# azrael417/mlperf-deepcam

Measured on AMD Instinct MI355X. Metric: samples/sec (768x1152x16) train step, higher is better.
Workload: dtype bf16; 1 GPU; DeepLabV3+/Xception train step (fwd + weighted CE + bwd + LAMB), 768x1152x16, local_batch=8, bf16 activations / fp32 master weights, random-init seed 333; local_batch=8, global_batch=8, parallelism=dp1, optimizer=LAMB, hip_graph=False, launch_list_replay=False

## Files before the change

mlperf-deepcam_amd/csrc/dwpipe.hip:

```cpp
#include "common.h"
#include "dwtile.h"
#include "dwtile_common.h"
#include "bn_fin.h"
#include "mfma_tile.h"

namespace dc {

namespace {

constexpr int P_TH = 8, P_TW = 8, P_CG = 16, P_THREADS = 512;
constexpr int P_ROWB = P_CG * 16;
constexpr int P_CH = P_CG * 8;

enum { PM_FLIP = 1, PM_STATS = 2, PM_WGRAD = 4, PM_ADD = 8, PM_XFORM = 16, PM_RES = 32, PM_MASK = 64 };

template <int DIL>
struct PCfg {
  static constexpr int HH = P_TH + 2 * DIL, HW = P_TW + 2 * DIL, HP = HH * HW;
  static constexpr int HIT = (HP * P_CG + P_THREADS - 1) / P_THREADS;
  static constexpr int HALO = HIT * P_THREADS * 16;
  static constexpr int LASTW = (HP * P_CG - (HIT - 1) * P_THREADS + 63) / 64;
  static constexpr int TILE = P_TH * P_TW * P_ROWB;
};

template <int DIL, int MODE>
struct PStage {
  static constexpr bool Y = (MODE & (PM_STATS | PM_WGRAD)) != 0, A = (MODE & PM_ADD) != 0, Y2 = (MODE & PM_RES) != 0;
  static constexpr int BYTES = PCfg<DIL>::HALO + ((Y ? 1 : 0) + (Y2 ? 1 : 0) + (A ? 1 : 0)) * PCfg<DIL>::TILE;
  static constexpr int DMAS = PCfg<DIL>::HIT + 2 * ((Y ? 1 : 0) + (Y2 ? 1 : 0) + (A ? 1 : 0));
  static constexpr int OFF_Y2 = PCfg<DIL>::HALO + (Y ? PCfg<DIL>::TILE : 0), OFF_A = OFF_Y2 + (Y2 ? PCfg<DIL>::TILE : 0);
  static constexpr int NS = (160 * 1024 / BYTES) > 4 ? 4 : (160 * 1024 / BYTES);
  static constexpr int STORES = DT_PX;
  static_assert(NS >= 2, "the ring needs two stages");
  static_assert((NS - 1) * STORES + (NS - 2) * DMAS < 64, "vmcnt immediate");
};

struct DwpArgs {
  const bf16* in;
  int ldin;
  const float* wp;
  const bf16* addend;
  int ldadd;
  bf16* out;
  int ldout;
  int H, W, C;
  int ncb, ntx, nty, ptiles;
  const float* pscale;
  const float* pshift;
  int prelu;
  DwBnStats st;
  const bf16* y2;
  int ldy2;
  const float* mean2;
  const float* invstd2;
  int relu2;
  float* slab2;
  int sum_row, sum_row2;
};

template <int N>
__device__ inline void wait_vm() {
  asm volatile("s_waitcnt vmcnt(%0)" ::"n"(N) : "memory");
}

template <int DIL, int MODE>
__global__ __launch_bounds__(P_THREADS) void dwp_kernel(const DwpArgs a) {
  typedef PCfg<DIL> K;
  typedef PStage<DIL, MODE> S;
  constexpr bool FLIP = (MODE & PM_FLIP) != 0, STATS = (MODE & PM_STATS) != 0, WGRAD = (MODE & PM_WGRAD) != 0, ADD = (MODE & PM_ADD) != 0,
                 XFORM = (MODE & PM_XFORM) != 0, RES = (MODE & PM_RES) != 0, MASK = (MODE & PM_MASK) != 0;
  static_assert(!RES || (WGRAD && !STATS), "PM_RES rides on the weight-gradient form");
  static_assert(!MASK || RES, "PM_MASK is a form of PM_RES");
  constexpr int WC = DT_PX + 2 * DIL, KH = 4, NS = S::NS;
  extern __shared__ __attribute__((aligned(16))) char smem[];
  const int tid = threadIdx.x;
  const int wv = __builtin_amdgcn_readfirstlane(tid >> 6);
  const int cb = blockIdx.x % a.ncb, wj = blockIdx.x / a.ncb, wc = gridDim.x / a.ncb;
  const int t0 = (int)((long)a.ptiles * wj / wc), t1 = (int)((long)a.ptiles * (wj + 1) / wc);
  const int nt = t1 - t0;
  const int ngroups = a.C >> 3, cg0 = cb * P_CG;
  const int H = a.H, W = a.W;
  const int h = tid & 31, sl = tid >> 5;
  const int row = sl >> 1, xs = (sl & 1) * DT_PX;
  const bool cok = cg0 + (h >> 1) < ngroups;
  const int ch0 = cok ? cg0 * 8 + h * KH : 0;
  const int g = tid & 15;
  const bool gok = cg0 + g < ngroups;
  constexpr unsigned OOB = 0x80000000u;
  unsigned hoff[K::HIT];
  unsigned hedge = 0;
#pragma unroll
  for (int it = 0; it < K::HIT; ++it) {
    const int hp = (it * P_THREADS + tid) >> 4;
    const int hy = hp / K::HW, hx = hp - hy * K::HW;
    hoff[it] = (gok && hp < K::HP) ? (unsigned)((((hy - DIL) * W + (hx - DIL)) * a.ldin + (cg0 + g) * 8) * 2) : OOB;
    hedge |= ((hx < DIL ? 1u : 0u) | (hx >= K::HW - DIL ? 2u : 0u)) << (2 * it);
  }
  unsigned yoff[2], aoff[2], y2off[2];
#pragma unroll
  for (int it = 0; it < 2; ++it) {
    const int pp = (it * P_THREADS + tid) >> 4;
    const int py = pp >> 3, px = pp & 7;
    yoff[it] = gok && S::Y ? (unsigned)(((py * W + px) * a.st.ldy + (cg0 + g) * 8) * 2) : OOB;
    aoff[it] = gok && S::A ? (unsigned)(((py * W + px) * a.ldadd + (cg0 + g) * 8) * 2) : OOB;
    y2off[it] = gok && S::Y2 ? (unsigned)(((py * W + px) * a.ldy2 + (cg0 + g) * 8) * 2) : OOB;
  }

  auto issue = [&](int t, int stage) {
#if defined(__HIP_DEVICE_COMPILE__)
    char* sb = smem + stage * S::BYTES;
    const bool live = t < t1;
    const int tt = live ? t : t0;
    const int tx = tt % a.ntx;
    const int r = tt / a.ntx;
    const int ty = r % a.nty, n = r / a.nty;
    const int y0 = ty * P_TH, x0 = tx * P_TW;
    const int live_mask = live ? -1 : 0;
    const unsigned emask = (x0 == 0 ? 0x55555555u : 0u) | (x0 + P_TW == W ? 0xAAAAAAAAu : 0u);
    {
      const __amdgpu_buffer_rsrc_t rs = __builtin_amdgcn_make_buffer_rsrc((void*)(a.in + (size_t)n * H * W * a.ldin), 0, (H * W * a.ldin * 2) & live_mask, 0x00020000);
      const unsigned torg = (unsigned)((y0 * W + x0) * a.ldin * 2);
#pragma unroll
      for (int it = 0; it < K::HIT; ++it) {
        if (it == K::HIT - 1 && wv >= K::LASTW) break;
        const unsigned vo = ((hedge & emask) >> (2 * it)) & 3u ? OOB : hoff[it] + torg;
        __builtin_amdgcn_raw_ptr_buffer_load_lds(rs, (lds_ptr)(sb + (it * P_THREADS + wv * 64) * 16), 16, vo, 0, 0, 0);
      }
    }
    if constexpr (S::Y) {
      const __amdgpu_buffer_rsrc_t rs = __builtin_amdgcn_make_buffer_rsrc((void*)(reinterpret_cast<const bf16*>(a.st.y) + (size_t)n * H * W * a.st.ldy), 0,
                                                                          (H * W * a.st.ldy * 2) & live_mask, 0x00020000);
      const unsigned torg = (unsigned)((y0 * W + x0) * a.st.ldy * 2);
#pragma unroll
      for (int it = 0; it < 2; ++it)
        __builtin_amdgcn_raw_ptr_buffer_load_lds(rs, (lds_ptr)(sb + K::HALO + (it * P_THREADS + wv * 64) * 16), 16, yoff[it] + torg, 0, 0, 0);
    }
    if constexpr (S::A) {
      const __amdgpu_buffer_rsrc_t rs = __builtin_amdgcn_make_buffer_rsrc((void*)(a.addend + (size_t)n * H * W * a.ldadd), 0, (H * W * a.ldadd * 2) & live_mask, 0x00020000);
      const unsigned torg = (unsigned)((y0 * W + x0) * a.ldadd * 2);
#pragma unroll
      for (int it = 0; it < 2; ++it)
        __builtin_amdgcn_raw_ptr_buffer_load_lds(rs, (lds_ptr)(sb + S::OFF_A + (it * P_THREADS + wv * 64) * 16), 16, aoff[it] + torg, 0, 0, 0);
    }
    if constexpr (S::Y2) {
      const __amdgpu_buffer_rsrc_t rs = __builtin_amdgcn_make_buffer_rsrc((void*)(a.y2 + (size_t)n * H * W * a.ldy2), 0, (H * W * a.ldy2 * 2) & live_mask, 0x00020000);
      const unsigned torg = (unsigned)((y0 * W + x0) * a.ldy2 * 2);
#pragma unroll
      for (int it = 0; it < 2; ++it)
        __builtin_amdgcn_raw_ptr_buffer_load_lds(rs, (lds_ptr)(sb + S::OFF_Y2 + (it * P_THREADS + wv * 64) * 16), 16, y2off[it] + torg, 0, 0, 0);
    }
#endif
  };

#pragma unroll
  for (int s = 0; s < NS - 1; ++s) issue(t0 + s, s);

  float wk[9][KH];
  load_taps<KH>(a.wp, ch0, a.C, FLIP, wk);
  BnAcc<KH> bn;
  if constexpr (STATS) bn.init(a.st, ch0);
  else if constexpr (WGRAD) bn.init_affine(a.st, ch0);
  float dwa[WGRAD ? 9 : 1][KH];
#pragma unroll
  for (int t9 = 0; t9 < (WGRAD ? 9 : 1); ++t9)
#pragma unroll
    for (int e = 0; e < KH; ++e) dwa[t9][e] = 0.f;
  float mu2[RES ? KH : 1], is2[RES ? KH : 1], ra[RES ? KH : 1], rb[RES ? KH : 1];
  if constexpr (RES) {
#pragma unroll
    for (int e = 0; e < KH; ++e) {
      mu2[e] = a.mean2[ch0 + e];
      is2[e] = a.invstd2[ch0 + e];
      ra[e] = rb[e] = 0.f;
      asm volatile("" : "+v"(mu2[e]), "+v"(is2[e]));
    }
  }
  float xsc[8], xsh[8];
  if constexpr (XFORM) {
#pragma unroll
    for (int e = 0; e < 8; ++e) {
      xsc[e] = gok ? a.pscale[(cg0 + g) * 8 + e] : 0.f;
      xsh[e] = gok ? a.pshift[(cg0 + g) * 8 + e] : 0.f;
    }
  }
#pragma unroll
  for (int t9 = 0; t9 < 9; ++t9)
#pragma unroll
    for (int e = 0; e < KH; ++e) asm volatile("" : "+v"(wk[t9][e]));
  if constexpr (STATS || WGRAD) {
#pragma unroll
    for (int e = 0; e < KH; ++e) asm volatile("" : "+v"(bn.mu[e]), "+v"(bn.is[e]), "+v"(bn.ms[e]), "+v"(bn.mh[e]));
  }
  if constexpr (XFORM) {
#pragma unroll
    for (int e = 0; e < 8; ++e) asm volatile("" : "+v"(xsc[e]), "+v"(xsh[e]));
  }
  auto decode = [&](int t, int& n, int& y0, int& x0) {
    const int tx = t % a.ntx;
    const int r = t / a.ntx;
    const int ty = r % a.nty;
    n = r / a.nty;
    y0 = ty * P_TH;
    x0 = tx * P_TW;
  };
  auto xform_tile = [&](int t, int stg) {
    char* sb = smem + stg * S::BYTES;
    int n, y0, x0;
    decode(t, n, y0, x0);
    (void)n;
#pragma unroll
      for (int it = 0; it < K::HIT; ++it) {
        if (it == K::HIT - 1 && wv >= K::LASTW) break;
        const int hp = (it * P_THREADS + tid) >> 4;
        const int hy = hp / K::HW, hx = hp - hy * K::HW;
        const int iy = y0 - DIL + hy, ix = x0 - DIL + hx;
        if (gok && hp < K::HP && (unsigned)iy < (unsigned)H && (unsigned)ix < (unsigned)W) {
          vec16* q = reinterpret_cast<vec16*>(sb) + it * P_THREADS + tid;
          float f[8];
          unpack(*q, f, bf16());
#pragma unroll
          for (int e = 0; e < 8; ++e) {
            const float v = fmaf(f[e], xsc[e], xsh[e]);
            f[e] = a.prelu ? fmaxf(v, 0.f) : v;
          }
          vec16 o;
          pack(o, f, bf16());
          typedef unsigned u32x4 __attribute__((ext_vector_type(4)));
          u32x4 ov;
          ov.x = o.w[0]; ov.y = o.w[1]; ov.z = o.w[2]; ov.w = o.w[3];
          const unsigned qa = (unsigned)(size_t)((__attribute__((address_space(3))) char*)reinterpret_cast<char*>(q));
          asm volatile("ds_write_b128 %0, %1" ::"v"(qa), "v"(ov) : "memory");
        }
      }
  };
  auto compute_tile = [&](int t, int stg) {
    char* sb = smem + stg * S::BYTES;
    int n, y0, x0;
    decode(t, n, y0, x0);
    const char* tile = sb + h * 8;
    const int oy = y0 + row;
    float yf[DT_PX][KH];
    if constexpr (S::Y) {
#pragma unroll
      for (int j = 0; j < DT_PX; ++j)
        unpack8(*reinterpret_cast<const vec8*>(sb + K::HALO + (row * P_TW + xs + j) * P_ROWB + h * 8), yf[j], bf16());
    }
    float xh[WGRAD ? DT_PX : 1][KH];
    if constexpr (WGRAD) {
#pragma unroll
      for (int j = 0; j < DT_PX; ++j) {
        float v[KH];
#pragma unroll
        for (int e = 0; e < KH; ++e) {
          const float u = fmaf(yf[j][e], bn.ms[e], bn.mh[e]);
          v[e] = a.st.relu ? fmaxf(u, 0.f) : u;
        }
        vec8 rr;
        pack8(rr, v, bf16());
        unpack8(rr, xh[j], bf16());
      }
    }
    float acc[DT_PX][KH];
#pragma unroll
    for (int j = 0; j < DT_PX; ++j)
#pragma unroll
      for (int e = 0; e < KH; ++e) acc[j][e] = 0.f;
#pragma unroll
    for (int ky = 0; ky < 3; ++ky) {
#pragma unroll
      for (int c = 0; c < WC; ++c) {
        float f[KH];
        unpack8(*reinterpret_cast<const vec8*>(tile + ((row + ky * DIL) * K::HW + xs + c) * P_ROWB), f, bf16());
#pragma unroll
        for (int kx = 0; kx < 3; ++kx) {
          const int j = c - kx * DIL;
          if (j >= 0 && j < DT_PX) {
#pragma unroll
            for (int e = 0; e < KH; ++e) acc[j][e] = fmaf(f[e], wk[ky * 3 + kx][e], acc[j][e]);
            if constexpr (WGRAD) {
#pragma unroll
              for (int e = 0; e < KH; ++e) dwa[8 - (ky * 3 + kx)][e] = fmaf(f[e], xh[j][e], dwa[8 - (ky * 3 + kx)][e]);
            }
          }
        }
      }
    }
#pragma unroll
    for (int j = 0; j < DT_PX; ++j) {
      if constexpr (ADD) {
        float av[KH];
        unpack8(*reinterpret_cast<const vec8*>(sb + S::OFF_A + (row * P_TW + xs + j) * P_ROWB + h * 8), av, bf16());
#pragma unroll
        for (int e = 0; e < KH; ++e) acc[j][e] += av[e];
      }
      if constexpr (MASK) {
#pragma unroll
        for (int e = 0; e < KH; ++e) acc[j][e] = yf[j][e] > 0.f ? acc[j][e] : 0.f;
      }
      vec8 v;
      pack8(v, acc[j], bf16());
      if (cok) *reinterpret_cast<vec8*>(a.out + (((size_t)n * H + oy) * W + x0 + xs + j) * a.ldout + ch0) = v;
      if constexpr (STATS) {
        float gs[KH];
        unpack8(v, gs, bf16());
        bn.add(gs, yf[j], a.st.relu);
      }
      if constexpr (RES) {
        float gs[KH], y2f[KH];
        unpack8(v, gs, bf16());
        unpack8(*reinterpret_cast<const vec8*>(sb + S::OFF_Y2 + (row * P_TW + xs + j) * P_ROWB + h * 8), y2f, bf16());
#pragma unroll
        for (int e = 0; e < KH; ++e) {
          const float gm = (MASK || !a.relu2 || yf[j][e] > 0.f) ? gs[e] : 0.f;
          ra[e] += gm;
          rb[e] = fmaf(gm, (y2f[e] - mu2[e]) * is2[e], rb[e]);
        }
      }
    }
  };
  int stage = 0;
  if constexpr (!XFORM) {
    for (int i = 0; i < nt; ++i) {
      if (wv < K::LASTW) {
        if (i >= NS - 1) wait_vm<(NS - 1) * S::STORES + (NS - 2) * S::DMAS>();
        else if (i == 0) wait_vm<(NS - 2) * S::DMAS>();
        else if (i == 1) wait_vm<S::STORES + (NS - 2) * S::DMAS>();
        else wait_vm<2 * S::STORES + (NS - 2) * S::DMAS>();
      } else {
        if (i >= NS - 1) wait_vm<(NS - 1) * S::STORES + (NS - 2) * (S::DMAS - 1)>();
        else if (i == 0) wait_vm<(NS - 2) * (S::DMAS - 1)>();
        else if (i == 1) wait_vm<S::STORES + (NS - 2) * (S::DMAS - 1)>();
        else wait_vm<2 * S::STORES + (NS - 2) * (S::DMAS - 1)>();
      }
      __builtin_amdgcn_s_barrier();
      {
        int ns = stage + NS - 1;
        if (ns >= NS) ns -= NS;
        issue(t0 + i + NS - 1, ns);
      }
      compute_tile(t0 + i, stage);
      if (++stage == NS) stage = 0;
    }
  } else {
    static_assert(!XFORM || NS >= 3, "the transform one tile ahead needs three stages");
    constexpr int D0 = S::DMAS, D1 = S::DMAS - 1;
    if (wv < K::LASTW) wait_vm<(NS - 2) * D0>(); else wait_vm<(NS - 2) * D1>();
    __builtin_amdgcn_s_barrier();
    xform_tile(t0, 0);
    for (int i = 0; i < nt; ++i) {
      if (wv < K::LASTW) {
        if (i >= NS - 2) wait_vm<(NS - 2) * S::STORES + (NS - 3) * D0>();
        else if (i == 0) wait_vm<(NS - 3) * D0>();
        else wait_vm<S::STORES + (NS - 3) * D0>();
      } else {
        if (i >= NS - 2) wait_vm<(NS - 2) * S::STORES + (NS - 3) * D1>();
        else if (i == 0) wait_vm<(NS - 3) * D1>();
        else wait_vm<S::STORES + (NS - 3) * D1>();
      }
      asm volatile("s_waitcnt lgkmcnt(0)" ::: "memory");
      __builtin_amdgcn_s_barrier();
      {
        int ns = stage + NS - 1;
        if (ns >= NS) ns -= NS;
        issue(t0 + i + NS - 1, ns);
      }
      if (i + 1 < nt) {
        int s1 = stage + 1;
        if (s1 == NS) s1 = 0;
        xform_tile(t0 + i + 1, s1);
      }
      compute_tile(t0 + i, stage);
      if (++stage == NS) stage = 0;
    }
  }
  wait_vm<0>();
  asm volatile("s_waitcnt lgkmcnt(0)" ::: "memory");
  __builtin_amdgcn_s_barrier();

  if constexpr (STATS) {
    float* red = reinterpret_cast<float*>(smem);
#pragma unroll
    for (int e = 0; e < KH; ++e) {
      red[(sl * 2 + 0) * P_CH + h * KH + e] = bn.a[e];
      red[(sl * 2 + 1) * P_CH + h * KH + e] = bn.b[e];
    }
    __syncthreads();
    if (tid < 2 * P_CH) {
      const int which = tid / P_CH, cl = tid % P_CH;
      const int c = cg0 * 8 + cl;
      if (c < a.C) {
        float s = 0.f;
#pragma unroll
        for (int q = 0; q < 16; ++q) s += red[(q * 2 + which) * P_CH + cl];
        if (a.sum_row) unsafeAtomicAdd(reinterpret_cast<double*>(a.st.slab) + (size_t)which * a.C + c, (double)s);
        else a.st.slab[((size_t)which * a.st.rows + wj) * a.C + c] = s;
      }
    }
    __syncthreads();
  }
  if constexpr (RES) {
    float* red = reinterpret_cast<float*>(smem);
#pragma unroll
    for (int e = 0; e < KH; ++e) {
      red[(sl * 2 + 0) * P_CH + h * KH + e] = ra[e];
      red[(sl * 2 + 1) * P_CH + h * KH + e] = rb[e];
    }
    __syncthreads();
    if (tid < 2 * P_CH) {
      const int which = tid / P_CH, cl = tid % P_CH;
      const int c = cg0 * 8 + cl;
      if (c < a.C) {
        float s = 0.f;
#pragma unroll
        for (int q = 0; q < 16; ++q) s += red[(q * 2 + which) * P_CH + cl];
        if (a.sum_row2) unsafeAtomicAdd(reinterpret_cast<double*>(a.slab2) + (size_t)which * a.C + c, (double)s);
        else a.slab2[((size_t)which * a.st.rows + wj) * a.C + c] = s;
      }
    }
    __syncthreads();
  }
  if constexpr (WGRAD) {
    float* red = reinterpret_cast<float*>(smem);
#pragma unroll
    for (int tp = 0; tp < 9; ++tp)
#pragma unroll
      for (int e = 0; e < KH; ++e) red[(sl * 9 + tp) * P_CH + h * KH + e] = dwa[tp][e];
    __syncthreads();
    for (int i = tid; i < 9 * P_CH; i += P_THREADS) {
      const int tp = i / P_CH, cl = i % P_CH;
      const int c = cg0 * 8 + cl;
      if (c < a.C) {
        float s = 0.f;
#pragma unroll
        for (int q = 0; q < 16; ++q) s += red[(q * 9 + tp) * P_CH + cl];
        a.st.wslab[((size_t)wj * 9 + tp) * a.C + c] = s;
      }
    }
  }
}

template <int DIL, int MODE>
int launch1(const DwpArgs& a, int grid, hipStream_t st) {
  constexpr int LDS = PStage<DIL, MODE>::NS * PStage<DIL, MODE>::BYTES;
  static_assert(LDS <= 160 * 1024, "ring larger than the LDS");
  static_assert(16 * 9 * P_CH * 4 <= LDS, "the fold's scratch lives in the drained ring");
  DC_ONCE((void)hipFuncSetAttribute(reinterpret_cast<const void*>(&dwp_kernel<DIL, MODE>), hipFuncAttributeMaxDynamicSharedMemorySize, LDS));
  hipLaunchKernelGGL((dwp_kernel<DIL, MODE>), dim3(grid), dim3(P_THREADS), LDS, st, a);
  DC_LAUNCHED((MODE & PM_MASK) ? "dwpipe_dgrad_masked" : (MODE & PM_FLIP) ? "dwpipe_dgrad" : "dwpipe_fwd");
  return 0;
}

}

bool dw_pipe_forward() { return g_options.dw_pipe == 2; }

int dw_pipe_rows(int dtype, int C, int dil, int N, int H, int W) {
  if (!g_options.dw_pipe || dtype != DC_BF16 || C < P_CH / 2 || (C & 7) || (H % P_TH) || (W % P_TW) || (dil != 1 && dil != 2)) return 0;
  if ((long)H * W * ((C + 63) / 64 * 64 + 64) * 2 >= (1L << 30)) return 0;
  const int ncb = cdiv(C / 8, P_CG);
  const long ptiles = (long)N * (H / P_TH) * (W / P_TW);
  long wc = 256 / ncb;
  if (wc < 1) wc = 1;
  if (wc > ptiles) wc = ptiles;
  const long rounds = (ptiles + wc - 1) / wc;
  wc = (ptiles + rounds - 1) / rounds;
  return (int)wc;
}

int launch_dw_pipe(int dil, bool flip, const void* in, int ldin, const float* wp, const void* addend, int ldadd, void* out, int ldout, int N,
                   int H, int W, int C, hipStream_t st, const float* pscale, const float* pshift, int prelu, const DwBnStats* bnstats,
                   const DwResStats* res) {
  const int wc = dw_pipe_rows(DC_BF16, C, dil, N, H, W);
  DC_REQUIRE(wc > 0, "launch_dw_pipe: shape not served");
  DwpArgs a;
  a.in = (const bf16*)in; a.ldin = ldin; a.wp = wp; a.addend = (const bf16*)addend; a.ldadd = ldadd; a.out = (bf16*)out; a.ldout = ldout;
  a.H = H; a.W = W; a.C = C;
  a.ncb = cdiv(C / 8, P_CG); a.ntx = W / P_TW; a.nty = H / P_TH; a.ptiles = N * a.ntx * a.nty;
  a.pscale = pscale; a.pshift = pshift; a.prelu = prelu;
  if (bnstats != nullptr) a.st = *bnstats;
  else { a.st.slab = nullptr; a.st.y = nullptr; a.st.ldy = 0; a.st.mean = a.st.invstd = a.st.mscale = a.st.mshift = nullptr; a.st.relu = 0; a.st.rows = 0; a.st.wslab = nullptr; }
  a.sum_row = bnstats != nullptr && bnstats->rows == SUM_ROW && bnstats->slab != nullptr;
  a.sum_row2 = res != nullptr && res->sum_row;
  a.st.rows = wc;
  a.y2 = nullptr; a.ldy2 = 0; a.mean2 = a.invstd2 = nullptr; a.relu2 = 0; a.slab2 = nullptr;
  if (res != nullptr) {
    a.y2 = (const bf16*)res->y; a.ldy2 = res->ldy; a.mean2 = res->mean; a.invstd2 = res->invstd; a.relu2 = res->relu; a.slab2 = res->slab;
  }
  const int grid = a.ncb * wc;
  const bool stats = flip && a.st.slab != nullptr, wg = flip && a.st.wslab != nullptr, add = flip && addend != nullptr;
  const bool xf = !flip && pscale != nullptr;
  DC_REQUIRE(!(stats || wg) || a.st.y != nullptr, "launch_dw_pipe: the sums need the BatchNorm input");
  if (res != nullptr) {
    DC_REQUIRE(wg && !stats && a.y2 && a.mean2 && a.invstd2 && a.slab2, "launch_dw_pipe: the residual BatchNorm's sums ride on the weight-gradient form");
    DC_REQUIRE(dil == 1, "launch_dw_pipe: the residual form is built for dilation 1 (with dilation 2 its ring would hold a single stage)");
    if (res->relu == 2) {
      if (add) return launch1<1, PM_FLIP | PM_WGRAD | PM_ADD | PM_RES | PM_MASK>(a, grid, st);
      return launch1<1, PM_FLIP | PM_WGRAD | PM_RES | PM_MASK>(a, grid, st);
    }
    if (add) return launch1<1, PM_FLIP | PM_WGRAD | PM_ADD | PM_RES>(a, grid, st);
    return launch1<1, PM_FLIP | PM_WGRAD | PM_RES>(a, grid, st);
  }
#define DWP(D, M) return launch1<D, M>(a, grid, st)
#define DWP_MODES(D)                                                                                      \
  if (!flip) { if (xf) DWP(D, PM_XFORM); else DWP(D, 0); }                                               \
  if (stats && wg) { if (add) DWP(D, PM_FLIP | PM_STATS | PM_WGRAD | PM_ADD); else DWP(D, PM_FLIP | PM_STATS | PM_WGRAD); } \
  if (stats) { if (add) DWP(D, PM_FLIP | PM_STATS | PM_ADD); else DWP(D, PM_FLIP | PM_STATS); }         \
  if (wg) { if (add) DWP(D, PM_FLIP | PM_WGRAD | PM_ADD); else DWP(D, PM_FLIP | PM_WGRAD); }            \
  if (add) DWP(D, PM_FLIP | PM_ADD); else DWP(D, PM_FLIP);
  if (dil == 1) { DWP_MODES(1) }
  DWP_MODES(2)
#undef DWP_MODES
#undef DWP
}

}
```

mlperf-deepcam_amd/csrc/dwtile_common.h:

```cpp
#pragma once
#include "common.h"

namespace dc {

constexpr int DT_PX = 4;

__device__ inline int xcd_remap(int bid, int nwg) {
  const int q8 = nwg >> 3, r8 = nwg & 7, xcd = bid & 7, slot = bid >> 3;
  return (xcd < r8 ? xcd * (q8 + 1) : r8 * (q8 + 1) + (xcd - r8) * q8) + slot;
}

struct alignas(8) vec8 {
  uint32_t w[2];
};
__device__ inline void unpack8(const vec8& v, float (&f)[2], float) {
  f[0] = __uint_as_float(v.w[0]);
  f[1] = __uint_as_float(v.w[1]);
}
__device__ inline void unpack8(const vec8& v, float (&f)[4], bf16) {
#pragma unroll
  for (int i = 0; i < 2; ++i) {
    f[2 * i] = __uint_as_float(v.w[i] << 16);
    f[2 * i + 1] = __uint_as_float(v.w[i] & 0xffff0000u);
  }
}
__device__ inline void pack8(vec8& v, const float (&f)[2], float) {
  v.w[0] = __float_as_uint(f[0]);
  v.w[1] = __float_as_uint(f[1]);
}
__device__ inline void pack8(vec8& v, const float (&f)[4], bf16) {
  v.w[0] = pack2_bf16(f[0], f[1]);
  v.w[1] = pack2_bf16(f[2], f[3]);
}

template <int KH>
__device__ inline void load_taps(const float* __restrict__ wp, int ch0, int C, bool flip, float (&wk)[9][KH]) {
#pragma unroll
  for (int t = 0; t < 9; ++t) {
    const float* src = wp + (size_t)(flip ? 8 - t : t) * C + ch0;
    if constexpr (KH == 4) {
      const float4 v = *reinterpret_cast<const float4*>(src);
      wk[t][0] = v.x; wk[t][1] = v.y; wk[t][2] = v.z; wk[t][3] = v.w;
    } else {
      const float2 v = *reinterpret_cast<const float2*>(src);
      wk[t][0] = v.x; wk[t][1] = v.y;
    }
  }
}


struct DwBnStats {
  const void* y;
  int ldy;
  const float* mean;
  const float* invstd;
  const float* mscale;
  const float* mshift;
  int relu;
  float* slab;
  int rows;
  float* wslab;
};

template <int KH>
struct BnAcc {
  float mu[KH], is[KH], ms[KH], mh[KH], a[KH], b[KH];
  __device__ inline void init(const DwBnStats& st, int ch0) {
    const bool affine = st.relu || st.wslab != nullptr;
#pragma unroll
    for (int e = 0; e < KH; ++e) {
      mu[e] = st.mean[ch0 + e];
      is[e] = st.invstd[ch0 + e];
      ms[e] = affine ? st.mscale[ch0 + e] : 0.f;
      mh[e] = affine ? st.mshift[ch0 + e] : 0.f;
      a[e] = b[e] = 0.f;
    }
  }
  __device__ inline void init_affine(const DwBnStats& st, int ch0) {
#pragma unroll
    for (int e = 0; e < KH; ++e) {
      mu[e] = is[e] = a[e] = b[e] = 0.f;
      ms[e] = st.mscale != nullptr ? st.mscale[ch0 + e] : 1.f;
      mh[e] = st.mshift != nullptr ? st.mshift[ch0 + e] : 0.f;
    }
  }
  __device__ inline void add(const float (&g)[KH], const float (&yv)[KH], int relu) {
#pragma unroll
    for (int e = 0; e < KH; ++e) {
      const float gm = (!relu || fmaf(yv[e], ms[e], mh[e]) > 0.f) ? g[e] : 0.f;
      a[e] += gm;
      b[e] = fmaf(gm, (yv[e] - mu[e]) * is[e], b[e]);
    }
  }
};

template <int KH, int NSL, int CW>
__device__ inline void bn_acc_store(float* red, const float (&a)[KH], const float (&b)[KH], bool cok, int h, int sl, const DwBnStats& st,
                                    int tile, int c_base, int C) {
  if (cok) {
#pragma unroll
    for (int e = 0; e < KH; ++e) {
      red[(sl * 2 + 0) * CW + h * KH + e] = a[e];
      red[(sl * 2 + 1) * CW + h * KH + e] = b[e];
    }
  }
  __syncthreads();
  for (int i = threadIdx.x; i < 2 * CW; i += 256) {
    const int which = i / CW, cl = i % CW;
    if (c_base + cl < C) {
      float s = 0.f;
#pragma unroll
      for (int q = 0; q < NSL; ++q) s += red[(q * 2 + which) * CW + cl];
      st.slab[((size_t)which * st.rows + tile) * C + c_base + cl] = s;
    }
  }
}

template <typename T, int HH, int HW, int CG>
__device__ inline void bn_transform_tile(char* smem, int iy0, int ix0, int H, int W, const float* __restrict__ pscale,
                                         const float* __restrict__ pshift, int prelu, int cg0, int ngroups, int cbase = 0) {
  constexpr int KPV = Elem<T>::kPerVec;
  constexpr int HP = HH * HW, ITER = (HP * CG + 255) / 256;
  const int tid = threadIdx.x, g = tid % CG;
  if (cg0 + g >= ngroups) return;
  float sc[KPV], sh[KPV];
#pragma unroll
  for (int e = 0; e < KPV; ++e) {
    sc[e] = pscale[(cg0 + g) * KPV + e - cbase];
    sh[e] = pshift[(cg0 + g) * KPV + e - cbase];
  }
#pragma unroll 2
  for (int it = 0; it < ITER; ++it) {
    const int slot = it * 256 + tid;
    const int hp = slot / CG;
    const int hy = hp / HW, hx = hp - hy * HW;
    const int iy = iy0 + hy, ix = ix0 + hx;
    if (hp < HP && (unsigned)iy < (unsigned)H && (unsigned)ix < (unsigned)W) {
      vec16* q = reinterpret_cast<vec16*>(smem) + slot;
      float f[KPV];
      unpack(*q, f, T());
#pragma unroll
      for (int e = 0; e < KPV; ++e) {
        const float v = fmaf(f[e], sc[e], sh[e]);
        f[e] = prelu ? fmaxf(v, 0.f) : v;
      }
      vec16 o;
      pack(o, f, T());
      *q = o;
    }
  }
}

}
```

Before: 261.4 samples/s.

## Cut per-tile integer and VALU overhead in depthwise pipeline kernel

Tile coordinates are now tracked incrementally rather than recomputed with divisions and modulos for each issue, xform and compute step. Per-row Y/A/Y2 offsets collapse to a single register with a row stride added at use. The inner accumulation uses packed f32x2 FMAs, ReLU/BN masks become SGPR ballot masks applied with v_cndmask, and LDS operands are preloaded. Loops are marked nounroll and a LEAN variant defers loads to limit register pressure. Together these aim to reduce VALU and scalar work in a memory-bound depthwise kernel, at the cost of extra inline asm and code complexity.

```diff
diff --git a/mlperf-deepcam_amd/csrc/dwpipe.hip b/mlperf-deepcam_amd/csrc/dwpipe.hip
--- a/mlperf-deepcam_amd/csrc/dwpipe.hip
+++ b/mlperf-deepcam_amd/csrc/dwpipe.hip
@@ -96,24 +96,38 @@
     hoff[it] = (gok && hp < K::HP) ? (unsigned)((((hy - DIL) * W + (hx - DIL)) * a.ldin + (cg0 + g) * 8) * 2) : OOB;
     hedge |= ((hx < DIL ? 1u : 0u) | (hx >= K::HW - DIL ? 2u : 0u)) << (2 * it);
   }
-  unsigned yoff[2], aoff[2], y2off[2];
-#pragma unroll
-  for (int it = 0; it < 2; ++it) {
-    const int pp = (it * P_THREADS + tid) >> 4;
+  unsigned yoff, aoff, y2off;
+  {
+    const int pp = tid >> 4;
     const int py = pp >> 3, px = pp & 7;
-    yoff[it] = gok && S::Y ? (unsigned)(((py * W + px) * a.st.ldy + (cg0 + g) * 8) * 2) : OOB;
-    aoff[it] = gok && S::A ? (unsigned)(((py * W + px) * a.ldadd + (cg0 + g) * 8) * 2) : OOB;
-    y2off[it] = gok && S::Y2 ? (unsigned)(((py * W + px) * a.ldy2 + (cg0 + g) * 8) * 2) : OOB;
-  }
+    yoff = gok && S::Y ? (unsigned)(((py * W + px) * a.st.ldy + (cg0 + g) * 8) * 2) : OOB;
+    aoff = gok && S::A ? (unsigned)(((py * W + px) * a.ldadd + (cg0 + g) * 8) * 2) : OOB;
+    y2off = gok && S::Y2 ? (unsigned)(((py * W + px) * a.ldy2 + (cg0 + g) * 8) * 2) : OOB;
+  }
+  constexpr int ROWS2 = P_THREADS / 16 / P_TW;
+
+  struct TilePos { int tx, ty, n; };
+  TilePos p0;
+  {
+    p0.tx = t0 % a.ntx;
+    const int r = t0 / a.ntx;
+    p0.ty = r % a.nty;
+    p0.n = r / a.nty;
+  }
+  auto advance = [&](TilePos& p) {
+    if (++p.tx == a.ntx) {
+      p.tx = 0;
+      if (++p.ty == a.nty) { p.ty = 0; ++p.n; }
+    }
+  };
+  TilePos pi = p0, px = p0, pc = p0;
 
   auto issue = [&](int t, int stage) {
 #if defined(__HIP_DEVICE_COMPILE__)
     char* sb = smem + stage * S::BYTES;
     const bool live = t < t1;
-    const int tt = live ? t : t0;
-    const int tx = tt % a.ntx;
-    const int r = tt / a.ntx;
-    const int ty = r % a.nty, n = r / a.nty;
+    const int tx = live ? pi.tx : 0, ty = live ? pi.ty : 0, n = live ? pi.n : 0;
+    advance(pi);
     const int y0 = ty * P_TH, x0 = tx * P_TW;
     const int live_mask = live ? -1 : 0;
     const unsigned emask = (x0 == 0 ? 0x55555555u : 0u) | (x0 + P_TW == W ? 0xAAAAAAAAu : 0u);
@@ -133,21 +147,21 @@
       const unsigned torg = (unsigned)((y0 * W + x0) * a.st.ldy * 2);
 #pragma unroll
       for (int it = 0; it < 2; ++it)
-        __builtin_amdgcn_raw_ptr_buffer_load_lds(rs, (lds_ptr)(sb + K::HALO + (it * P_THREADS + wv * 64) * 16), 16, yoff[it] + torg, 0, 0, 0);
+        __builtin_amdgcn_raw_ptr_buffer_load_lds(rs, (lds_ptr)(sb + K::HALO + (it * P_THREADS + wv * 64) * 16), 16, yoff + (torg + (unsigned)(it * ROWS2 * W * a.st.ldy * 2)), 0, 0, 0);
     }
     if constexpr (S::A) {
       const __amdgpu_buffer_rsrc_t rs = __builtin_amdgcn_make_buffer_rsrc((void*)(a.addend + (size_t)n * H * W * a.ldadd), 0, (H * W * a.ldadd * 2) & live_mask, 0x00020000);
       const unsigned torg = (unsigned)((y0 * W + x0) * a.ldadd * 2);
 #pragma unroll
       for (int it = 0; it < 2; ++it)
-        __builtin_amdgcn_raw_ptr_buffer_load_lds(rs, (lds_ptr)(sb + S::OFF_A + (it * P_THREADS + wv * 64) * 16), 16, aoff[it] + torg, 0, 0, 0);
+        __builtin_amdgcn_raw_ptr_buffer_load_lds(rs, (lds_ptr)(sb + S::OFF_A + (it * P_THREADS + wv * 64) * 16), 16, aoff + (torg + (unsigned)(it * ROWS2 * W * a.ldadd * 2)), 0, 0, 0);
     }
     if constexpr (S::Y2) {
       const __amdgpu_buffer_rsrc_t rs = __builtin_amdgcn_make_buffer_rsrc((void*)(a.y2 + (size_t)n * H * W * a.ldy2), 0, (H * W * a.ldy2 * 2) & live_mask, 0x00020000);
       const unsigned torg = (unsigned)((y0 * W + x0) * a.ldy2 * 2);
 #pragma unroll
       for (int it = 0; it < 2; ++it)
-        __builtin_amdgcn_raw_ptr_buffer_load_lds(rs, (lds_ptr)(sb + S::OFF_Y2 + (it * P_THREADS + wv * 64) * 16), 16, y2off[it] + torg, 0, 0, 0);
+        __builtin_amdgcn_raw_ptr_buffer_load_lds(rs, (lds_ptr)(sb + S::OFF_Y2 + (it * P_THREADS + wv * 64) * 16), 16, y2off + (torg + (unsigned)(it * ROWS2 * W * a.ldy2 * 2)), 0, 0, 0);
     }
 #endif
   };
@@ -195,19 +209,10 @@
 #pragma unroll
     for (int e = 0; e < 8; ++e) asm volatile("" : "+v"(xsc[e]), "+v"(xsh[e]));
   }
-  auto decode = [&](int t, int& n, int& y0, int& x0) {
-    const int tx = t % a.ntx;
-    const int r = t / a.ntx;
-    const int ty = r % a.nty;
-    n = r / a.nty;
-    y0 = ty * P_TH;
-    x0 = tx * P_TW;
-  };
-  auto xform_tile = [&](int t, int stg) {
+  auto xform_tile = [&](int stg) {
     char* sb = smem + stg * S::BYTES;
-    int n, y0, x0;
-    decode(t, n, y0, x0);
-    (void)n;
+    const int y0 = px.ty * P_TH, x0 = px.tx * P_TW;
+    advance(px);
 #pragma unroll
       for (int it = 0; it < K::HIT; ++it) {
         if (it == K::HIT - 1 && wv >= K::LASTW) break;
@@ -233,38 +238,69 @@
         }
       }
   };
-  auto compute_tile = [&](int t, int stg) {
+  const unsigned ooff = (unsigned)(((row * W + xs) * a.ldout + ch0) * 2), ldob = (unsigned)(a.ldout * 2);
+  auto compute_tile = [&](int stg) {
     char* sb = smem + stg * S::BYTES;
-    int n, y0, x0;
-    decode(t, n, y0, x0);
+    const int n = pc.n, y0 = pc.ty * P_TH, x0 = pc.tx * P_TW;
+    advance(pc);
+    char* ob = reinterpret_cast<char*>(a.out + (((size_t)n * H + y0) * W + x0) * a.ldout);
     const char* tile = sb + h * 8;
-    const int oy = y0 + row;
+    const char* own = sb + (row * P_TW + xs) * P_ROWB + h * 8;
+    constexpr bool LEAN = DIL == 2 && STATS && WGRAD;
     float yf[DT_PX][KH];
+    f32x2 yu[(STATS || WGRAD) ? DT_PX : 1][KH / 2];
+    wave_mask pos[(STATS || RES) ? DT_PX : 1][KH];
     if constexpr (S::Y) {
 #pragma unroll
-      for (int j = 0; j < DT_PX; ++j)
-        unpack8(*reinterpret_cast<const vec8*>(sb + K::HALO + (row * P_TW + xs + j) * P_ROWB + h * 8), yf[j], bf16());
+      for (int j = 0; j < DT_PX; ++j) {
+        unpack8(*reinterpret_cast<const vec8*>(own + K::HALO + j * P_ROWB), yf[j], bf16());
+        if constexpr (STATS || WGRAD) {
+#pragma unroll
+          for (int e = 0; e < KH; e += 2) yu[j][e >> 1] = fma2(yf[j], bn.ms, bn.mh, e);
+        }
+        if constexpr (STATS && !(LEAN && ADD)) {
+#pragma unroll
+          for (int e = 0; e < KH; ++e) pos[j][e] = mask_gt0(yu[j][e >> 1][e & 1], a.st.relu ? 0ull : ~0ull);
+        }
+        if constexpr (RES) {
+#pragma unroll
+          for (int e = 0; e < KH; ++e) pos[j][e] = mask_gt0(yf[j][e], (MASK || a.relu2) ? 0ull : ~0ull);
+        }
+      }
+    }
+    vec8 avp[ADD ? DT_PX : 1], y2p[RES ? DT_PX : 1];
+    if constexpr (ADD && !LEAN) {
+#pragma unroll
+      for (int j = 0; j < DT_PX; ++j) avp[j] = *reinterpret_cast<const vec8*>(own + S::OFF_A + j * P_ROWB);
+    }
+    if constexpr (RES) {
+#pragma unroll
+      for (int j = 0; j < DT_PX; ++j) y2p[j] = *reinterpret_cast<const vec8*>(own + S::OFF_Y2 + j * P_ROWB);
     }
     float xh[WGRAD ? DT_PX : 1][KH];
     if constexpr (WGRAD) {
-#pragma unroll
-      for (int j = 0; j < DT_PX; ++j) {
-        float v[KH];
-#pragma unroll
-        for (int e = 0; e < KH; ++e) {
-          const float u = fmaf(yf[j][e], bn.ms[e], bn.mh[e]);
-          v[e] = a.st.relu ? fmaxf(u, 0.f) : u;
-        }
-        vec8 rr;
-        pack8(rr, v, bf16());
-        unpack8(rr, xh[j], bf16());
-      }
-    }
-    float acc[DT_PX][KH];
+      f32x2 v[DT_PX][KH / 2];
+#pragma unroll
+      for (int j = 0; j < DT_PX; ++j)
+#pragma unroll
+        for (int p = 0; p < KH / 2; ++p) v[j][p] = yu[j][p];
+      if (a.st.relu) {
+        asm volatile("");
+#pragma unroll
+        for (int j = 0; j < DT_PX; ++j)
+#pragma unroll
+          for (int p = 0; p < KH / 2; ++p) v[j][p] = f32x2{relu_f32(v[j][p][0]), relu_f32(v[j][p][1])};
+      }
+#pragma unroll
+      for (int j = 0; j < DT_PX; ++j)
+#pragma unroll
+        for (int p = 0; p < KH / 2; ++p) round2_bf16(v[j][p][0], v[j][p][1], xh[j][2 * p], xh[j][2 * p + 1]);
+    }
+    f32x2 acc2[DT_PX][KH / 2];
 #pragma unroll
     for (int j = 0; j < DT_PX; ++j)
 #pragma unroll
-      for (int e = 0; e < KH; ++e) acc[j][e] = 0.f;
+      for (int p = 0; p < KH / 2; ++p) acc2[j][p] = f32x2{0.f, 0.f};
 #pragma unroll
     for (int ky = 0; ky < 3; ++ky) {
 #pragma unroll
@@ -273,45 +309,73 @@
         unpack8(*reinterpret_cast<const vec8*>(tile + ((row + ky * DIL) * K::HW + xs + c) * P_ROWB), f, bf16());
 #pragma unroll
         for (int kx = 0; kx < 3; ++kx) {
-          const int j = c - kx * DIL;
+          const int j = c - kx * DIL, t9 = ky * 3 + kx;
           if (j >= 0 && j < DT_PX) {
 #pragma unroll
-            for (int e = 0; e < KH; ++e) acc[j][e] = fmaf(f[e], wk[ky * 3 + kx][e], acc[j][e]);
+            for (int p = 0; p < KH / 2; ++p) {
+              const f32x2 fv = {f[2 * p], f[2 * p + 1]};
+              acc2[j][p] = __builtin_elementwise_fma(fv, f32x2{wk[t9][2 * p], wk[t9][2 * p + 1]}, acc2[j][p]);
+            }
             if constexpr (WGRAD) {
 #pragma unroll
-              for (int e = 0; e < KH; ++e) dwa[8 - (ky * 3 + kx)][e] = fmaf(f[e], xh[j][e], dwa[8 - (ky * 3 + kx)][e]);
+              for (int e = 0; e < KH; ++e) dwa[8 - t9][e] = fmaf(f[e], xh[j][e], dwa[8 - t9][e]);
             }
           }
         }
       }
     }
+    float acc[DT_PX][KH];
+#pragma unroll
+    for (int j = 0; j < DT_PX; ++j)
+#pragma unroll
+      for (int e = 0; e < KH; ++e) acc[j][e] = acc2[j][e >> 1][e & 1];
+    typedef __attribute__((address_space(3))) const char lds_cchar;
+    lds_cchar* own2 = (lds_cchar*)own;
+    if constexpr (LEAN) asm("" : "+v"(own2));
 #pragma unroll
     for (int j = 0; j < DT_PX; ++j) {
       if constexpr (ADD) {
         float av[KH];
-        unpack8(*reinterpret_cast<const vec8*>(sb + S::OFF_A + (row * P_TW + xs + j) * P_ROWB + h * 8), av, bf16());
-#pragma unroll
-        for (int e = 0; e < KH; ++e) acc[j][e] += av[e];
+        if constexpr (LEAN) avp[j] = *reinterpret_cast<const vec8*>(own + S::OFF_A + j * P_ROWB);
+        unpack8(avp[j], av, bf16());
+#pragma unroll
+        for (int p = 0; p < KH / 2; ++p) {
+          const f32x2 s2 = acc2[j][p] + f32x2{av[2 * p], av[2 * p + 1]};
+          acc[j][2 * p] = s2[0];
+          acc[j][2 * p + 1] = s2[1];
+        }
       }
       if constexpr (MASK) {
 #pragma unroll
-        for (int e = 0; e < KH; ++e) acc[j][e] = yf[j][e] > 0.f ? acc[j][e] : 0.f;
+        for (int e = 0; e < KH; ++e) acc[j][e] = masked(pos[j][e], acc[j][e]);
       }
       vec8 v;
       pack8(v, acc[j], bf16());
-      if (cok) *reinterpret_cast<vec8*>(a.out + (((size_t)n * H + oy) * W + x0 + xs + j) * a.ldout + ch0) = v;
+      if (cok) *reinterpret_cast<vec8*>(ob + (ooff + (unsigned)j * ldob)) = v;
       if constexpr (STATS) {
+        if constexpr (LEAN) {
+          const unsigned long long y2w = *reinterpret_cast<__attribute__((address_space(3))) const unsigned long long*>(own2 + K::HALO + j * P_ROWB);
+          vec8 yv;
+          yv.w[0] = (uint32_t)y2w;
+          yv.w[1] = (uint32_t)(y2w >> 32);
+          unpack8(yv, yf[j], bf16());
+        }
         float gs[KH];
         unpack8(v, gs, bf16());
-        bn.add(gs, yf[j], a.st.relu);
+#pragma unroll
+        for (int e = 0; e < KH; ++e) {
+          const float gm = (LEAN && ADD) ? ((!a.st.relu || fmaf(yf[j][e], bn.ms[e], bn.mh[e]) > 0.f) ? gs[e] : 0.f) : masked(pos[j][e], gs[e]);
+          bn.a[e] += gm;
+          bn.b[e] = fmaf(gm, (yf[j][e] - bn.mu[e]) * bn.is[e], bn.b[e]);
+        }
       }
       if constexpr (RES) {
         float gs[KH], y2f[KH];
         unpack8(v, gs, bf16());
-        unpack8(*reinterpret_cast<const vec8*>(sb + S::OFF_Y2 + (row * P_TW + xs + j) * P_ROWB + h * 8), y2f, bf16());
+        unpack8(y2p[j], y2f, bf16());
 #pragma unroll
         for (int e = 0; e < KH; ++e) {
-          const float gm = (MASK || !a.relu2 || yf[j][e] > 0.f) ? gs[e] : 0.f;
+          const float gm = MASK ? gs[e] : masked(pos[j][e], gs[e]);
           ra[e] += gm;
           rb[e] = fmaf(gm, (y2f[e] - mu2[e]) * is2[e], rb[e]);
         }
@@ -320,6 +384,7 @@
   };
   int stage = 0;
   if constexpr (!XFORM) {
+#pragma nounroll
     for (int i = 0; i < nt; ++i) {
       if (wv < K::LASTW) {
         if (i >= NS - 1) wait_vm<(NS - 1) * S::STORES + (NS - 2) * S::DMAS>();
@@ -338,7 +403,7 @@
         if (ns >= NS) ns -= NS;
         issue(t0 + i + NS - 1, ns);
       }
-      compute_tile(t0 + i, stage);
+      compute_tile(stage);
       if (++stage == NS) stage = 0;
     }
   } else {
@@ -346,7 +411,8 @@
     constexpr int D0 = S::DMAS, D1 = S::DMAS - 1;
     if (wv < K::LASTW) wait_vm<(NS - 2) * D0>(); else wait_vm<(NS - 2) * D1>();
     __builtin_amdgcn_s_barrier();
-    xform_tile(t0, 0);
+    xform_tile(0);
+#pragma nounroll
     for (int i = 0; i < nt; ++i) {
       if (wv < K::LASTW) {
         if (i >= NS - 2) wait_vm<(NS - 2) * S::STORES + (NS - 3) * D0>();
@@ -367,9 +433,9 @@
       if (i + 1 < nt) {
         int s1 = stage + 1;
         if (s1 == NS) s1 = 0;
-        xform_tile(t0 + i + 1, s1);
-      }
-      compute_tile(t0 + i, stage);
+        xform_tile(s1);
+      }
+      compute_tile(stage);
       if (++stage == NS) stage = 0;
     }
   }
diff --git a/mlperf-deepcam_amd/csrc/dwtile_common.h b/mlperf-deepcam_amd/csrc/dwtile_common.h
--- a/mlperf-deepcam_amd/csrc/dwtile_common.h
+++ b/mlperf-deepcam_amd/csrc/dwtile_common.h
@@ -31,6 +31,38 @@
 __device__ inline void pack8(vec8& v, const float (&f)[4], bf16) {
   v.w[0] = pack2_bf16(f[0], f[1]);
   v.w[1] = pack2_bf16(f[2], f[3]);
+}
+
+__device__ inline void round2_bf16(float lo, float hi, float& rlo, float& rhi) {
+  uint32_t w = pack2_bf16(lo, hi);
+  asm("" : "+v"(w));
+  rlo = __uint_as_float(w << 16);
+  rhi = __uint_as_float(w & 0xffff0000u);
+}
+
+typedef float f32x2 __attribute__((ext_vector_type(2)));
+template <int KH>
+__device__ inline f32x2 fma2(const float (&x)[KH], const float (&s)[KH], const float (&t)[KH], int e) {
+  const f32x2 xv = {x[e], x[e + 1]}, sv = {s[e], s[e + 1]}, tv = {t[e], t[e + 1]};
+  return __builtin_elementwise_fma(xv, sv, tv);
+}
+
+__device__ inline float relu_f32(float x) {
+  float r;
+  asm("v_max_f32 %0, 0, %1" : "=v"(r) : "v"(x));
+  return r;
+}
+
+typedef unsigned long long wave_mask;
+__device__ inline wave_mask mask_gt0(float x, wave_mask always = 0) {
+  wave_mask m = __builtin_amdgcn_ballot_w64(x > 0.f) | always;
+  asm("" : "+s"(m));
+  return m;
+}
+__device__ inline float masked(wave_mask m, float g) {
+  float r;
+  asm("v_cndmask_b32_e64 %0, 0, %1, %2" : "=v"(r) : "v"(g), "s"(m));
+  return r;
 }
 
 template <int KH>
```

Measured after the change: 264.3 samples/s, median of 6. 1.01x the previous value.
